# jhhung/kISS

Hardware: AMD Instinct MI355X
Metric: bases/sec suffix_sort (chm13v2.0-size synthetic, k=256) (higher is better)
Workload: dtype u8; 1 GPU; suffix_sort genome-like synthetic n=3117292070 k=256 (stand-in for chm13v2.0.fa, BASELINE.json configs[1]); PARALLEL_SORTING; text resident in HBM, SA left in HBM; n=3117292070, k=256, seed=2, parallelism=single GPU, lms=905939973, lms_rounds=9, tied_after_round0_item_rounds=184319413, big_segment_item_rounds=72866550, workspace_bytes=80357006484, induce_passes=47

## Files before the change

### kiss_amd/csrc/api.hip

```cpp
#include "kiss_internal.hpp"
#include <cstdlib>
#include <chrono>
#include <mutex>
#include <cstring>
#include <new>

KTimer::KTimer(kiss_hip_ctx *c, int cls, uint64_t items) : ctx(c), idx(-1)
{
    if (!((ctx->profile_mask >> cls) & 1ull)) return;
    if (ctx->ev_used == ctx->ev_pool.size()) {
        kiss_hip_ctx::Ev e;
        if (hipEventCreate(&e.a) != hipSuccess || hipEventCreate(&e.b) != hipSuccess) return;
        e.cls = 0;
        ctx->ev_pool.push_back(e);
    }
    idx = (int)ctx->ev_used++;
    ctx->ev_pool[idx].cls = cls;
    ctx->stats.launches_kernel[cls]++;
    ctx->stats.items_kernel[cls] += items;
    (void)hipEventRecord(ctx->ev_pool[idx].a, ctx->stream);
}
KTimer::~KTimer()
{
    if (idx >= 0) (void)hipEventRecord(ctx->ev_pool[idx].b, ctx->stream);
}
void ktimer_collect(kiss_hip_ctx *ctx)
{
    for (size_t i = 0; i < ctx->ev_used; i++) {
        float ms = 0.f;
        if (hipEventElapsedTime(&ms, ctx->ev_pool[i].a, ctx->ev_pool[i].b) == hipSuccess)
            ctx->stats.ms_kernel[ctx->ev_pool[i].cls] += ms;
    }
    ctx->ev_used = 0;
}

static void kiss_opts_supported_from_env(KissOpts &o)
{
    o.debug = getenv("KISS_HIP_DEBUG") != nullptr;
    if (const char *e = getenv("KISS_HIP_XFER_THREADS")) o.xfer_threads = atoi(e);
    if (const char *e = getenv("KISS_HIP_PREFAULT_THREADS")) o.prefault_threads = atoi(e);
}
#ifdef KISS_HIP_HOOKS
static bool env_on(const char *name) { return getenv(name) != nullptr; }
static unsigned long long env_u64(const char *name, unsigned long long dflt)
{
    const char *e = getenv(name);
    return e ? strtoull(e, nullptr, 0) : dflt;
}
void kiss_opts_refresh(kiss_hip_ctx *ctx)
{
    KissOpts o;
    kiss_opts_supported_from_env(o);
    if (const char *e = getenv("KISS_HIP_SYNC_READBACK")) o.sync_readback = atoi(e) != 0;
    o.no_serialize = env_on("KISS_HIP_NO_SERIALIZE");
    o.no_lms_exact = env_on("KISS_HIP_NO_LMS_EXACT");
    o.heads_by_compare = env_on("KISS_HIP_LMS_HEADS_BY_COMPARE");
    o.no_early_out = env_on("KISS_HIP_NO_EARLY_OUT");
    o.no_pivot_rounds = env_on("KISS_HIP_NO_PIVOT_ROUNDS");
    o.pivot_from_round2 = env_on("KISS_HIP_PIVOT_FROM_ROUND2");
    o.pair_keys = env_on("KISS_HIP_PAIR_KEYS");
    o.no_fc0_onepass = env_on("KISS_HIP_NO_FC0_ONEPASS");
    o.no_pair_records = env_on("KISS_HIP_NO_PAIR_RECORDS");
    o.no_small_fused = env_on("KISS_HIP_NO_SMALL_FUSED");
    o.no_class_bytes = env_on("KISS_HIP_NO_CLASS_BYTES");
    o.no_pivot_ctx = env_on("KISS_HIP_NO_PIVOT_CTX");
    o.no_taint = env_on("KISS_HIP_NO_TAINT");
    o.isa_direct = env_on("KISS_HIP_ISA_DIRECT");
    o.no_onesweep = env_on("KISS_HIP_NO_ONESWEEP");
    o.rx_one_tile = env_on("KISS_HIP_RX_ONE_TILE");
    o.merge_lms = env_on("KISS_HIP_MERGE_LMS");
    o.no_small_alphabet = env_on("KISS_HIP_NO_SMALL_ALPHABET");
    o.induce_one_pass = env_on("KISS_HIP_INDUCE_ONE_PASS");
    o.verify = env_on("KISS_HIP_VERIFY");
    o.no_prefault = env_on("KISS_HIP_NO_PREFAULT");
    o.doubling_h0 = (uint32_t)env_u64("KISS_HIP_DOUBLING_H0", 0);
    o.tcap0 = env_u64("KISS_HIP_TCAP0", 0);
    o.pivot_slots = (int)env_u64("KISS_HIP_PIVOT_SLOTS", 3);
    o.small_seg = (uint32_t)env_u64("KISS_HIP_SMALL_SEG", 0);
    o.near_merge_min = (uint32_t)env_u64("KISS_HIP_NEAR_MERGE_MIN", 4096);
    o.induce_small_max = (uint32_t)env_u64("KISS_HIP_INDUCE_SMALL_MAX", 0);
    o.collapse_cap = (uint32_t)env_u64("KISS_HIP_COLLAPSE_CAP", 0);
    o.collapse_n = env_u64("KISS_HIP_COLLAPSE_N", 0);
    o.fm_heavy = (uint32_t)env_u64("KISS_HIP_FM_HEAVY", 0);
    o.fm_light = (uint32_t)env_u64("KISS_HIP_FM_LIGHT", 0);
    o.fm_mm_wave = env_on("KISS_HIP_FM_MM_WAVE");
    o.fm_mm_budget = env_u64("KISS_HIP_FM_MM_BUDGET", 0);
    o.fm8_group = env_on("KISS_HIP_FM8_GROUP");
    o.isa_direct_max = env_u64("KISS_HIP_ISA_DIRECT_MAX", 0);
    o.lx_sync_points = (unsigned)env_u64("KISS_HIP_LX_SYNC_POINTS", 0);
    o.tie_trace = (unsigned)env_u64("KISS_HIP_TIE_TRACE", 0);
    o.poison = (uint32_t)env_u64("KISS_HIP_POISON", 0);
    if (const char *e = getenv("KISS_HIP_DUMP_PIVOT")) snprintf(o.dump_pivot, sizeof o.dump_pivot, "%s", e);
    ctx->opts = o;
}
static std::mutex &kiss_launch_mutex()
// ... 760 lines not shown
        }
    }
    return KISS_HIP_OK;
}

int kiss_hip_debug_radix_sort(kiss_hip_ctx *ctx, uint64_t *keys, uint32_t *pos, uint64_t count, int key_lo_bit)
{
    if (!ctx || !keys || !pos || count > ctx->m_cap) return KISS_HIP_E_INVALID;
    KCHECK(hipSetDevice(ctx->device));
    KCHECK(hipMemcpy(ctx->keyA, keys, count * 8, hipMemcpyHostToDevice));
    KCHECK(hipMemcpy(ctx->posA, pos, count * 4, hipMemcpyHostToDevice));
    RadixBufs rb = kiss_ctx_radix_bufs(ctx);
    int res = 0;
    KTRY(kiss_radix_sort(ctx, rb, count, key_lo_bit, 0, &res));
    KTRY(kiss_radix_check(ctx));
    ktimer_collect(ctx);
    KCHECK(hipMemcpy(keys, rb.key[res], count * 8, hipMemcpyDeviceToHost));
    KCHECK(hipMemcpy(pos, rb.pos[res], count * 4, hipMemcpyDeviceToHost));
    return KISS_HIP_OK;
}

int kiss_hip_debug_fail_alloc_over(kiss_hip_ctx *ctx, uint64_t bytes)
{
    if (!ctx) return KISS_HIP_E_INVALID;
#ifdef KISS_HIP_HOOKS
    ctx->fail_alloc_over = bytes;
    return KISS_HIP_OK;
#else
    (void)bytes;
    return KISS_HIP_E_UNSUPPORTED;
#endif
}

int kiss_hip_has_hooks(void)
{
#ifdef KISS_HIP_HOOKS
    return 1;
#else
    return 0;
#endif
}

int kiss_hip_debug_scan_u32(kiss_hip_ctx *ctx, uint32_t *data, uint64_t count)
{
    if (!ctx || !data || count > ctx->m_cap) return KISS_HIP_E_INVALID;
    KCHECK(hipSetDevice(ctx->device));
    KCHECK(hipMemcpy(ctx->posA, data, count * 4, hipMemcpyHostToDevice));
    KTRY(kiss_scan_u32(ctx, ctx->posA, ctx->posB, count));
    KCHECK(hipStreamSynchronize(ctx->stream));
    KCHECK(hipMemcpy(data, ctx->posB, count * 4, hipMemcpyDeviceToHost));
    return KISS_HIP_OK;
}

int kiss_hip_ctx_get_stage_outputs(kiss_hip_ctx *ctx, uint32_t *lms_ascending, uint32_t *lms_sorted, uint64_t *counts)
{
    if (!ctx) return KISS_HIP_E_INVALID;
    KCHECK(hipSetDevice(ctx->device));
    if (lms_ascending && ctx->m)
        KCHECK(hipMemcpy(lms_ascending, ctx->lms_pos, ctx->m * sizeof(uint32_t), hipMemcpyDeviceToHost));
    if (lms_sorted && ctx->m) {
        KTRY(kiss_merge_lms(ctx));
        KCHECK(hipStreamSynchronize(ctx->stream));
    }
    if (lms_sorted && ctx->m)
        KCHECK(hipMemcpy(lms_sorted, ctx->lmsP, ctx->m * sizeof(uint32_t), hipMemcpyDeviceToHost));
    if (counts)
// ... 22 lines not shown
```

### kiss_amd/csrc/kiss_internal.hpp

```cpp
#pragma once
#include <hip/hip_runtime.h>
#include <stdint.h>
#include <stddef.h>
#include <mutex>
#include <vector>
#include "../../include/kiss_hip.h"

struct KissOpts {
    bool debug = false;
    int xfer_threads = 0;
    int prefault_threads = 0;
    bool sync_readback = false;
    bool no_lms_exact = false;
    bool heads_by_compare = false;
    bool no_early_out = false;
    bool no_pivot_rounds = false;
    bool pivot_from_round2 = false;
    bool pair_keys = false;
    bool no_fc0_onepass = false;
    bool no_pair_records = false;
    bool no_small_fused = false;
    bool no_class_bytes = false;
    bool no_pivot_ctx = false;
    bool no_taint = false;
    bool isa_direct = false;
    bool no_onesweep = false;
    bool rx_one_tile = false;
    bool merge_lms = false;
    bool no_small_alphabet = false;
    bool induce_one_pass = false;
    bool verify = false;
    bool no_prefault = false;
    bool no_serialize = false;
    bool lock_launches = false;
    bool sync_launches = false;
    uint32_t doubling_h0 = 0;
    uint64_t tcap0 = 0;
    int pivot_slots = 3;
    uint32_t small_seg = 0;
    uint32_t near_merge_min = 4096;
    uint32_t induce_small_max = 0;
    uint32_t collapse_cap = 0;
    uint64_t collapse_n = 0;
    uint32_t fm_heavy = 0, fm_light = 0;
    bool fm_mm_wave = false;
    bool fm8_group = false;
    uint64_t fm_mm_budget = 0;
    uint64_t isa_direct_max = 0;
    unsigned lx_sync_points = 0;
    unsigned tie_trace = 0;
    uint32_t poison = 0;
    char dump_pivot[256] = {0};
};
// ... 159 lines not shown
    uint32_t ind_ticket_base = 0;
    uint32_t *d_small = nullptr;
    uint32_t *h_pinned = nullptr;
    uint32_t *h_pub = nullptr;
    uint32_t *d_pub = nullptr;
    uint32_t pub_seq = 0;
    int pub_mode = -1;
    uint64_t *pairs1 = nullptr, *pairs2 = nullptr;
    uint64_t pairs_cap = 0;
    void *fm_pool[FM_SLOT_COUNT] = {};
    uint64_t fm_pool_cap[FM_SLOT_COUNT] = {};
    hipEvent_t fm_ev[6] = {};
    uint32_t *near_idx = nullptr, *near_fin = nullptr, *near_pos = nullptr, *near_tmp = nullptr, *near_tmp2 = nullptr;
    uint64_t near_cap = 0;
    uint8_t *ga_codes = nullptr;
    uint64_t ga_codes_cap = 0;
    uint8_t *refine_heads = nullptr;
    uint8_t *hfar = nullptr, *hmerged = nullptr;
    uint32_t h_depth = 0;
    bool lms_merged = false;
    int near_form = 0;
    const uint32_t *near_sorted = nullptr;
    const uint32_t *rm_fin = nullptr, *rm_pos = nullptr;
    uint32_t rm_E = 0;

    uint8_t *io_S = nullptr;
    uint32_t *io_SA = nullptr;
    uint64_t io_cap = 0;
    uint32_t *early_host_SA = nullptr;
    hipStream_t early_stream = nullptr;
    std::vector<hipEvent_t> early_events;
    size_t early_used = 0;
    uint64_t early_bytes = 0;
    void *xf_pin[16][2] = {};
    hipEvent_t xf_done[16][2] = {};
    hipStream_t xf_stream[16] = {};
    int xf_ready = 0;

    uint64_t n = 0, m = 0, m_far = 0;
    uint64_t counts[12] = {0};
    kiss_hip_stats stats{};
    uint64_t profile_mask = 0;
    struct Ev { hipEvent_t a, b; int cls; };
    std::vector<Ev> ev_pool;
    size_t ev_used = 0;
};

void kiss_drain_deferred(kiss_hip_ctx *ctx);
struct KissOwnStreamAtExit {
    kiss_hip_ctx *ctx;
    explicit KissOwnStreamAtExit(kiss_hip_ctx *c) : ctx(c) {}
    ~KissOwnStreamAtExit()
    {
        if (ctx) ctx->stream = ctx->own_stream;
    }
    KissOwnStreamAtExit(const KissOwnStreamAtExit &) = delete;
    KissOwnStreamAtExit &operator=(const KissOwnStreamAtExit &) = delete;
};
struct KissCallStream : KissOwnStreamAtExit {
    KissCallStream(kiss_hip_ctx *c, void *stream) : KissOwnStreamAtExit(c)
    {
        ctx->stream = stream ? (hipStream_t)stream : ctx->own_stream;
        if (!ctx->deferred_free.empty()) kiss_drain_deferred(ctx);
    }
};

struct KTimer {
    kiss_hip_ctx *ctx;
    int idx;
    KTimer(kiss_hip_ctx *c, int cls, uint64_t items);
    ~KTimer();
};
void ktimer_collect(kiss_hip_ctx *ctx);

static inline uint64_t div_up(uint64_t a, uint64_t b) { return (a + b - 1) / b; }

int kiss_lms_reserve(kiss_hip_ctx *ctx, uint64_t m_cap, uint64_t t_cap_wanted = 0, bool defer_frees = false);
int kiss_lms_reserve_deferred(kiss_hip_ctx *ctx, uint64_t m_cap);
int kiss_tied_reserve(kiss_hip_ctx *ctx, uint64_t t_cap);
int kiss_workspace_ready(kiss_hip_ctx *ctx);
int kiss_need_ctx_words(kiss_hip_ctx *ctx);
int kiss_pack_text(kiss_hip_ctx *ctx, const uint8_t *d_S, uint64_t n);
int kiss_classify(kiss_hip_ctx *ctx, uint64_t n, uint64_t depth , uint64_t win_lo, uint64_t win_hi);
int kiss_readback(kiss_hip_ctx *ctx, const void *d_src, uint32_t nwords);
std::mutex &kiss_device_mutex(int device);
int kiss_scan_u32(kiss_hip_ctx *ctx, const uint32_t *in, uint32_t *out, uint64_t count);
int kiss_scan_u64(kiss_hip_ctx *ctx, const uint64_t *in, uint64_t *out, uint64_t count);
int kiss_zero_u32(kiss_hip_ctx *ctx, void *p, uint64_t count_u32);
int kiss_fill_u32(kiss_hip_ctx *ctx, void *p, uint32_t value, uint64_t count_u32);
struct RadixBufs {
    uint64_t *key[2];
    uint32_t *seg[2];
    uint32_t *pos[2];
    const uint32_t *first_pos = nullptr;
};
static inline RadixBufs kiss_ctx_radix_bufs(kiss_hip_ctx *ctx)
{
    RadixBufs b;
    b.key[0] = ctx->keyA;
    b.key[1] = ctx->keyB;
    b.seg[0] = b.seg[1] = nullptr;
    b.pos[0] = ctx->posA;
    b.pos[1] = ctx->posB;
// ... 11 lines not shown
constexpr uint32_t KISS_EXACT_H0 = 512;
int kiss_exact_refine(kiss_hip_ctx *ctx, uint64_t n, uint32_t h0, uint32_t *d_SA, uint8_t *heads_in = nullptr);
int kiss_isa_build(kiss_hip_ctx *ctx, const uint32_t *SA, uint64_t total, uint32_t *isa);
int kiss_rank_build_lms(kiss_hip_ctx *ctx, const uint32_t *L, const uint32_t *lms_asc, uint64_t m, uint64_t n,
                        uint32_t *rank, uint64_t *pairs1, uint64_t *pairs2, uint32_t *small, uint64_t small_words);
int kiss_lms_exact_refine(kiss_hip_ctx *ctx, uint64_t n, uint32_t h0, uint32_t *scratch, bool *resolved);
int kiss_merge_lms(kiss_hip_ctx *ctx);
#ifdef KISS_HIP_HOOKS
void kiss_tie_trace_report(kiss_hip_ctx *ctx);
#endif
int kiss_place_lms(kiss_hip_ctx *ctx, uint64_t n, uint32_t k, uint64_t depth);
int kiss_xfer_h2d(kiss_hip_ctx *ctx, void *d_dst, const void *h_src, uint64_t bytes);
int kiss_io_reserve(kiss_hip_ctx *ctx, uint64_t n);
int kiss_cached_ctx_run(int device, uint64_t n, int (*fn)(kiss_hip_ctx *, void *), void *arg);
template <class F>
static inline int kiss_one_shot_cached(int device, uint64_t max_n, const F &f)
{
    return kiss_cached_ctx_run(device, max_n, [](kiss_hip_ctx *ctx, void *p) { return (*static_cast<const F *>(p))(ctx); }, (void *)&f);
}
template <class F>
static inline int kiss_one_shot_own(int device, uint64_t max_n, const F &f)
{
    kiss_hip_ctx *ctx = nullptr;
    int rc = kiss_hip_ctx_create(&ctx, device, max_n);
    if (rc) return rc;
    rc = f(ctx);
    kiss_hip_ctx_destroy(ctx);
    return rc;
}
int kiss_xfer_d2h(kiss_hip_ctx *ctx, void *h_dst, const void *d_src, uint64_t bytes);
void kiss_xfer_free(kiss_hip_ctx *ctx);
int kiss_induce(kiss_hip_ctx *ctx, uint64_t n, uint32_t *d_SA);
int kiss_early_out(kiss_hip_ctx *ctx, const uint32_t *d_SA, uint64_t lo, uint64_t hi);

#ifdef __HIPCC__
__device__ __forceinline__ void kiss_words2(const uint64_t *__restrict__ pk, uint64_t w, uint64_t &a, uint64_t &b)
{
    const uint64_t w0 = w & ~1ull;
    const ulonglong2 ab = *reinterpret_cast<const ulonglong2 *>(__builtin_assume_aligned(pk + w0, 16));
    const uint64_t c = pk[w0 + 2];
    const bool odd = (w & 1ull) != 0;
    a = odd ? ab.y : ab.x;
    b = odd ? c : ab.y;
}
__device__ __forceinline__ void kiss_words5(const uint64_t *__restrict__ pk, uint64_t w, uint64_t x[5])
{
    const uint64_t w0 = w & ~1ull;
    const ulonglong2 p0 = *reinterpret_cast<const ulonglong2 *>(__builtin_assume_aligned(pk + w0, 16));
    const ulonglong2 p1 = *reinterpret_cast<const ulonglong2 *>(__builtin_assume_aligned(pk + w0 + 2, 16));
    const ulonglong2 p2 = *reinterpret_cast<const ulonglong2 *>(__builtin_assume_aligned(pk + w0 + 4, 16));
    const bool odd = (w & 1ull) != 0;
    x[0] = odd ? p0.y : p0.x;
    x[1] = odd ? p1.x : p0.y;
    x[2] = odd ? p1.y : p1.x;
    x[3] = odd ? p2.x : p1.y;
    x[4] = odd ? p2.y : p2.x;
}
__device__ __forceinline__ uint64_t kiss_key32(const uint64_t *__restrict__ pk, uint64_t p)
{
    const uint32_t s = (uint32_t)(p & 31u) * 2u;
    uint64_t a, b;
    kiss_words2(pk, p >> 5, a, b);
    return (a << s) | ((b >> 1) >> (63u - s));
}
__device__ __forceinline__ uint32_t kiss_base(const uint64_t *__restrict__ pk, uint64_t p)
{
// ... 39 lines not shown
```

### kiss_amd/csrc/lms_sort.hip

```cpp
#include "flag_compact.hpp"
#include <cstdio>
#include <vector>

using namespace kiss_fc;

namespace {

constexpr uint32_t LMS_SMALL_SEG = 24;
constexpr int ROUND0_BASES = 20;

__global__ __launch_bounds__(LS_THREADS) void k_gather_keys(const uint64_t *__restrict__ pk, uint64_t n,
                                                           const uint32_t *__restrict__ pos, uint64_t count,
                                                           uint64_t depth_off, uint64_t mask,
                                                           uint64_t *__restrict__ key, const uint32_t *__restrict__ seg,
                                                           const uint32_t *__restrict__ segstart, uint32_t min_len,
                                                           uint32_t max_len)
{
    uint64_t i = (uint64_t)blockIdx.x * LS_THREADS + threadIdx.x;
    if (i >= count) return;
    if (seg) {
        const uint32_t sg = seg[i];
        const uint32_t len = segstart[sg + 1] - segstart[sg];
        if (len < min_len || len > max_len) return;
    }
// ... 313 lines not shown
    const int wa = s_a[w], wb = s_b[w];
    uint32_t r;
    bool taint, tied_before;
    if (!s_unsorted[w]) {
        r = (uint32_t)(w - wa);
        tied_before = w > wa && s_inorder[w - 1] == 2;
        taint = tied_before || (w + 1 < wb && s_inorder[w] == 2);
    } else {
        const uint32_t behind = (2u << (wb - 1 - w)) - 2u;
        r = (uint32_t)__popc(~s_before[w] & behind);
        taint = s_tiedm[w] != 0;
        tied_before = false;
        for (int j = wa; j < w; j++) {
            r += (s_before[j] >> (w - j)) & 1u;
            tied_before = tied_before || ((s_tiedm[j] >> (w - j)) & 1u);
        }
        taint = taint || tied_before;
    }
    const uint32_t dst = slot[my_a + r];
    out[dst] = s_pos[w];
    if (hfar && tied_before) hfar[dst] = 0;
    if (tctx) octx[dst] = tctx[i] | (taint ? KISS_CTX_TAINT : 0u);
    else if (taint) octx[dst] = KISS_CTX_TAINT;
    big[i] = 0;
}

__global__ __launch_bounds__(LS_THREADS) void k_pair_finish(const uint64_t *__restrict__ pk, uint64_t n,
                                                           const uint32_t *__restrict__ rpos0,
                                                           const uint32_t *__restrict__ rpos1,
                                                           const uint32_t *__restrict__ rslot, uint64_t npairs,
                                                           uint64_t off, uint64_t depth, uint32_t *__restrict__ out,
                                                           uint32_t *__restrict__ octx, uint8_t *__restrict__ hfar)
{
    const uint64_t i = (uint64_t)blockIdx.x * LS_THREADS + threadIdx.x;
    if (i >= npairs) return;
    const uint32_t p0 = rpos0[i], p1 = rpos1[i], s = rslot[i];
    bool taint = false;
    const bool swap = deep_less(pk, n, p1, p0, off - 32, depth, false, &taint);
    if (!swap && !taint) return;
    const uint32_t c0 = octx[s], c1 = octx[s + 1];
    const uint32_t t = taint ? KISS_CTX_TAINT : 0u;
    if (swap) {
        out[s] = p1;
        out[s + 1] = p0;
    }
    octx[s] = (swap ? c1 : c0) | t;
    octx[s + 1] = (swap ? c0 : c1) | t;
    if (hfar && taint) hfar[s + 1] = 0;
}

__device__ __forceinline__ uint32_t pivot_class(const uint64_t *__restrict__ bkey, uint32_t a, uint32_t b, uint64_t k)
{
    const uint64_t pv = bkey[(a + b) >> 1];
    return k < pv ? 0u : (k == pv ? 1u : 2u);
}

__global__ __launch_bounds__(LS_THREADS) void k_pivot_class(const uint64_t *__restrict__ bkey,
                                                           const uint32_t *__restrict__ bseg,
                                                           const uint32_t *__restrict__ bsegstart, uint64_t nbig,
                                                           uint64_t *__restrict__ cls)
{
    const uint64_t i = (uint64_t)blockIdx.x * LS_THREADS + threadIdx.x;
    if (i >= nbig) return;
    const uint32_t sid = bseg[i];
    const uint32_t c = pivot_class(bkey, bsegstart[sid], bsegstart[sid + 1], bkey[i]);
    cls[i] = c == 0 ? 1ull : (c == 1 ? (1ull << 32) : 0ull);
}

__global__ __launch_bounds__(LS_THREADS) void k_pivot_scatter(const uint64_t *__restrict__ bkey,
                                                             const uint32_t *__restrict__ bpos,
                                                             const uint32_t *__restrict__ bseg,
                                                             const uint32_t *__restrict__ bsegstart, uint64_t nbig,
                                                             const uint64_t *__restrict__ cls,
                                                             const uint64_t *__restrict__ ex,
                                                             const uint64_t *__restrict__ tot,
                                                             uint64_t *__restrict__ okey, uint32_t *__restrict__ opos,
                                                             uint64_t *__restrict__ ne)
{
    const uint64_t i = (uint64_t)blockIdx.x * LS_THREADS + threadIdx.x;
    if (i >= nbig) return;
    const uint32_t sid = bseg[i];
// ... 83 lines not shown
        complete = true;
    }
    key <<= (uint64_t)slotbits * (uint64_t)(slots - used);
    key = (key << 1) | (complete ? 1ull : 0ull);
    keyout[i] = (key << (64 - (slots * slotbits + 1))) | (with_ctx ? (uint64_t)kiss_load_ctx_n(pk, bpos[i], KISS_KEY_CTX_BASES) : 0ull);
}

__global__ __launch_bounds__(LS_THREADS) void k_pivot_heads(const uint64_t *__restrict__ key,
                                                           const uint32_t *__restrict__ seg, uint64_t nbig,
                                                           int complete_bit, uint8_t *__restrict__ heads,
                                                           uint64_t cmp_mask)
{
    const uint64_t i = (uint64_t)blockIdx.x * LS_THREADS + threadIdx.x;
    if (i >= nbig) return;
    const uint64_t k = key[i] & cmp_mask;
    const bool complete = ((k >> complete_bit) & 1ull) != 0;
    const bool same_prev = i > 0 && seg[i] == seg[i - 1] && (key[i - 1] & cmp_mask) == k;
    uint8_t h = 1;
    if (same_prev && !complete) h = 0;
    if (complete && (same_prev || (i + 1 < nbig && seg[i + 1] == seg[i] && (key[i + 1] & cmp_mask) == k))) h |= 2;
    if (complete && same_prev) h |= 4;
    heads[i] = h;
}

__global__ void k_ctx_lengths_anchor(const uint64_t *pk, uint32_t *out)
{
    out[threadIdx.x] = kiss_load_ctx(pk, out[threadIdx.x + 64]);
}


struct LmsViews {
    uint32_t *rpos0, *rpos1, *rslot;
    uint64_t rcol;
    uint64_t *K1;
    uint64_t *key2;
    uint64_t *F1, *F2;
    uint8_t *pivot_heads;
    uint32_t *seg2, *bss;
    uint32_t *sortpos[2];
    uint32_t *tctx, *bslot;
    uint64_t *d_total, *d_ptot;
    uint32_t *d_nbig;
};

LmsViews views_of(kiss_hip_ctx *ctx)
{
    LmsViews v;
    v.rcol = (ctx->m_far / 2 + 4) & ~3ull;
    v.rpos0 = reinterpret_cast<uint32_t *>(ctx->keyA);
    v.rpos1 = v.rpos0 + v.rcol;
    v.rslot = v.rpos1 + v.rcol;
    v.K1 = ctx->keyA;
    v.key2 = ctx->keyB;
    v.F1 = ctx->flags;
    v.F2 = ctx->flags + ctx->t_cap;
    v.pivot_heads = reinterpret_cast<uint8_t *>(ctx->segB);
    v.seg2 = ctx->segB;
    v.bss = ctx->segstartB;
    v.sortpos[0] = ctx->lmsP;
    v.sortpos[1] = ctx->lmsC;
    v.tctx = v.bslot = ctx->bslot;
    v.d_total = reinterpret_cast<uint64_t *>(ctx->d_small + 2);
    v.d_nbig = ctx->d_small + 8;
    v.d_ptot = reinterpret_cast<uint64_t *>(ctx->d_small + 24);
    return v;
}

struct LmsSort {
    kiss_hip_ctx *ctx;
    uint64_t n, depth;
    bool dbg;
    bool pivot_on;
    bool pivot_r1;
    int pivot_slots;
    bool no_pair_keys;
    uint32_t small_seg;
    bool small_fused;
    LmsViews v;
    uint32_t *Pc, *Sc, *Gc, *SSc;
    uint64_t count, nseg;
    uint64_t off = ROUND0_BASES;
    uint64_t npairs = 0;
    bool have_tctx = false;
    bool first_refine = true;
    unsigned pivot_rounds_done = 0;

    FcOut survivors() const { return FcOut{Pc, Sc, Gc, SSc}; }
    void take_tied_arrays()
    {
        Sc = ctx->slotA;
        Gc = ctx->segA;
        SSc = ctx->segstartA;
        v = views_of(ctx);
    }
    void set_survivors(uint64_t tot)
    {
        count = tot >> 32;
        nseg = tot & 0xFFFFFFFFull;
    }
};

struct Round {
// ... 56 lines not shown
            if ((tot >> 32) <= ctx->t_cap) break;
            if (attempt) return KINTERNAL();
            KTRY(regrow_tied(s, tot >> 32));
        }
        s.have_tctx = true;
    } else {
        FcJob job;
        job.key = rb.key[res];
        job.pos = rb.pos[res];
        job.count = count;
        job.cmp_shift = r0_shift;
        job.out = ctx->lms_sorted_far;
        job.octx = ctx->lms_ctx_far;
        KTRY(fc_count(ctx, job, s.v.d_total));
        KTRY(read_u64(ctx, s.v.d_total, &tot));
        if ((tot >> 32) > ctx->t_cap) {
            KTRY(regrow_tied(s, tot >> 32));
            KTRY(fc_count(ctx, job, s.v.d_total));
        }
        job.nctx = s.v.tctx;
        KTRY(fc_compact(ctx, job, s.survivors(), &s.have_tctx));
    }
    s.set_survivors(tot);
    if (s.dbg)
        fprintf(stderr, "[kiss_hip] round 0: items %llu -> survivors %llu in %llu segments\n", (unsigned long long)count,
                (unsigned long long)s.count, (unsigned long long)s.nseg);
    return KISS_HIP_OK;
}

int finish_pair_records(LmsSort &s)
{
    kiss_hip_ctx *ctx = s.ctx;
    if (s.npairs > ctx->m_far / 2) return KINTERNAL();
    {
        KTimer t(ctx, KISS_HIP_K_SEGRANK, 2 * s.npairs);
        hipLaunchKernelGGL(k_pair_finish, dim3((unsigned)div_up(s.npairs, LS_THREADS)), dim3(LS_THREADS), 0, ctx->stream, ctx->pk, s.n,
                           s.v.rpos0, s.v.rpos1, s.v.rslot, s.npairs, (uint64_t)ROUND0_BASES, s.depth, ctx->lms_sorted_far,
                           ctx->lms_ctx_far, ctx->hfar);
        KCHECK(hipGetLastError());
    }
    ctx->stats.pair_records = (uint32_t)s.npairs;
    ctx->stats.sort_item_rounds += 2 * s.npairs;
    if (s.count == 0) ctx->stats.lms_rounds++;
    return KISS_HIP_OK;
}

int gather_keys(LmsSort &s, const Round &r)
{
    kiss_hip_ctx *ctx = s.ctx;
    if (s.small_fused && r.pivot_ahead) return KISS_HIP_OK;
    const uint32_t *seg = s.Gc;
    uint32_t min_len = s.small_seg + 1u, max_len = 0xFFFFFFFFu;
    if (!s.small_fused) {
        seg = s.no_pair_keys ? s.Gc : (const uint32_t *)nullptr;
        min_len = 3u;
        max_len = r.pivot_ahead ? s.small_seg : 0xFFFFFFFFu;
    }
    KTimer t(ctx, KISS_HIP_K_KEYGATHER, s.count);
    set_u32(ctx, s.SSc + s.nseg, (uint32_t)s.count);
    hipLaunchKernelGGL(k_gather_keys, dim3(r.grid), dim3(LS_THREADS), 0, ctx->stream, ctx->pk, s.n, s.Pc, s.count, s.off, r.mask,
                       s.v.K1, seg, s.SSc, min_len, max_len);
    KCHECK(hipGetLastError());
    return KISS_HIP_OK;
}

int finish_small_segments(LmsSort &s, const Round &r)
{
    kiss_hip_ctx *ctx = s.ctx;
    {
        KTimer t(ctx, KISS_HIP_K_SEGRANK, s.count);
        set_u32(ctx, s.SSc + s.nseg, (uint32_t)s.count, s.v.d_nbig);
        const uint32_t *tctx = (s.have_tctx && s.first_refine) ? s.v.tctx : (const uint32_t *)nullptr;
        if (s.small_fused) {
            hipLaunchKernelGGL(k_small_finish, dim3(r.grid), dim3(SF_THREADS), 0, ctx->stream, ctx->pk, s.n, s.Pc, s.Sc, s.Gc, s.SSc,
                               (uint32_t)s.count, s.off, s.depth, r.mask, ctx->lms_sorted_far, r.bigb, tctx, ctx->lms_ctx_far,
                               ctx->hfar);
        } else {
            hipLaunchKernelGGL(k_seg_adjacent, dim3(r.grid), dim3(LS_THREADS), 0, ctx->stream, ctx->pk, s.n, s.v.K1, s.Pc, s.Gc,
                               s.SSc, s.count, s.off, s.depth, s.small_seg, r.inorder);
            hipLaunchKernelGGL(k_seg_finish, dim3(r.grid), dim3(LS_THREADS), 0, ctx->stream, ctx->pk, s.n, s.v.K1, s.Pc, s.Sc, s.Gc,
                               s.SSc, s.count, s.off, s.depth, s.small_seg, r.inorder, ctx->lms_sorted_far, r.bigb, s.v.d_nbig,
                               tctx, ctx->lms_ctx_far, ctx->hfar);
        }
        KCHECK(hipGetLastError());
    }
    ctx->stats.lms_rounds++;
    ctx->stats.sort_item_rounds += s.count;
    return KISS_HIP_OK;
}

int compact_big_segments(LmsSort &s, const Round &r, uint64_t nbig, uint64_t nbigseg)
{
    kiss_hip_ctx *ctx = s.ctx;
    const BigbOut to{ctx->bkeyA, ctx->bposA, ctx->bsegA, s.v.bslot, s.v.bss};
// ... 189 lines not shown
    hipStream_t stream;
    hipEvent_t e0 = nullptr, e1 = nullptr;
    DbgSpan(kiss_hip_ctx *ctx, bool on) : stream(ctx->stream)
    {
        if (!on) return;
        (void)hipEventCreate(&e0);
        (void)hipEventCreate(&e1);
        (void)hipEventRecord(e0, stream);
    }
    float ms()
    {
        float v = 0;
        (void)hipEventRecord(e1, stream);
        (void)hipEventSynchronize(e1);
        (void)hipEventElapsedTime(&v, e0, e1);
        return v;
    }
    ~DbgSpan()
    {
        if (e0) (void)hipEventDestroy(e0);
        if (e1) (void)hipEventDestroy(e1);
    }
};

}

int kiss_lms_sort(kiss_hip_ctx *ctx, uint64_t n, uint32_t k, uint64_t depth)
{
    (void)k;
    const uint64_t m_far = ctx->m_far;
    ctx->stats.lms_rounds = 0;
    ctx->stats.sort_item_rounds = 0;
    ctx->stats.pair_records = 0;
    if (m_far == 0) return KISS_HIP_OK;
    if (m_far == 1) {
        KCHECK(hipMemcpyAsync(ctx->lms_sorted_far, ctx->lms_pos, sizeof(uint32_t), hipMemcpyDeviceToDevice,
                              ctx->stream));
        KTRY(kiss_zero_u32(ctx, ctx->lms_ctx_far, 1));
        return KISS_HIP_OK;
    }
    LmsSort s;
    s.ctx = ctx;
    s.n = n;
    s.depth = depth;
    s.dbg = ctx->opts.debug;
    s.pivot_on = !ctx->opts.no_pivot_rounds;
    s.pivot_r1 = !ctx->opts.pivot_from_round2;
    s.pivot_slots = ctx->opts.pivot_slots >= 1 && ctx->opts.pivot_slots <= 8 ? ctx->opts.pivot_slots : 3;
    s.no_pair_keys = !ctx->opts.pair_keys;
    s.small_seg = ctx->opts.small_seg >= 2 && ctx->opts.small_seg <= 4096 ? ctx->opts.small_seg : LMS_SMALL_SEG;
    s.small_fused = !ctx->opts.no_small_fused && s.small_seg == LMS_SMALL_SEG;
    s.take_tied_arrays();

    KTRY(round0(s));
    if (s.npairs) KTRY(finish_pair_records(s));

    for (;; s.first_refine = false) {
        if (s.count == 0) break;
        if (depth && s.off >= depth) return KINTERNAL();
        const Round r = round_of(s);
        KTRY(gather_keys(s, r));
        uint64_t bt;
        {
            DbgSpan span(ctx, s.dbg);
            KTRY(finish_small_segments(s, r));
            KTRY(bigb_count(ctx, r.bigb, s.count, s.v.d_total, &bt));
            if (s.dbg) fprintf(stderr, "[kiss_hip]   seg_finish + flag scan %.3f ms\n", span.ms());
        }
        const uint64_t nbig = bt >> 32, nbigseg = bt & 0xFFFFFFFFull;
        if (s.dbg)
            fprintf(stderr, "[kiss_hip] round off=%llu: items %llu in %llu segments, big-segment items %llu\n",
                    (unsigned long long)s.off, (unsigned long long)s.count, (unsigned long long)s.nseg, (unsigned long long)nbig);
        if (nbig == 0) break;
        KTRY(compact_big_segments(s, r, nbig, nbigseg));
        if (r.pivot_ahead) {
            KTRY(pivot_round(s, nbig, nbigseg));
            continue;
        }
        SortedBig sorted;
        if (uint64_t *NE = class_split_flags(s, nbig)) KTRY(class_split_round(s, r, NE, nbig, nbigseg, &sorted));
        else KTRY(radix_round(s, r, nbig, nbigseg, &sorted));
        KTRY(closing_compaction(s, r, sorted, nbig));
        s.off += 32;
        if (!depth && s.off > n + 64 && s.count > 0) return KINTERNAL();
        if (!depth && s.off >= KISS_EXACT_MSD_MAX_DEPTH && s.count > 0) return KISS_INTERNAL_TOO_DEEP;
    }
    return KISS_HIP_OK;
}
```

### kiss_amd/csrc/xfer.hip

```cpp
#include "kiss_internal.hpp"
#include <atomic>
#include <cstdlib>
#include <cstring>
#include <new>
#include <thread>
#include <vector>

namespace {

constexpr int XF_MAX_THREADS = 16;
static int xf_threads(const kiss_hip_ctx *ctx)
{
    const int v = ctx->opts.xfer_threads ? ctx->opts.xfer_threads : 8;
    return v < 1 ? 1 : (v > XF_MAX_THREADS ? XF_MAX_THREADS : v);
}
#define XF_THREADS xf_threads(ctx)
constexpr size_t XF_CHUNK = 16ull << 20;

bool host_is_pinned(const void *p)
{
    hipPointerAttribute_t a;
    std::memset(&a, 0, sizeof a);
    if (hipPointerGetAttributes(&a, p) != hipSuccess) {
        (void)hipGetLastError();
// ... 86 lines not shown
            th.emplace_back(work, t);
        } catch (...) {
            orphan.push_back(t);
        }
    }
    if (threads > 0) work(0);
    for (int t : orphan) work(t);
    for (auto &x : th) x.join();
    return status;
}

}

int kiss_early_out(kiss_hip_ctx *ctx, const uint32_t *d_SA, uint64_t lo, uint64_t hi)
{
    if (!ctx->early_host_SA || hi <= lo) return KISS_HIP_OK;
    if (!ctx->early_stream) KCHECK(hipStreamCreateWithFlags(&ctx->early_stream, hipStreamNonBlocking));
    if (ctx->early_used == ctx->early_events.size()) {
        hipEvent_t e;
        KCHECK(hipEventCreateWithFlags(&e, hipEventDisableTiming));
        ctx->early_events.push_back(e);
    }
    hipEvent_t ev = ctx->early_events[ctx->early_used++];
    KCHECK(hipEventRecord(ev, ctx->stream));
    KCHECK(hipStreamWaitEvent(ctx->early_stream, ev, 0));
    KCHECK(hipMemcpyAsync(ctx->early_host_SA + lo, d_SA + lo, (hi - lo) * sizeof(uint32_t), hipMemcpyDeviceToHost,
                          ctx->early_stream));
    ctx->early_bytes += (hi - lo) * sizeof(uint32_t);
    return KISS_HIP_OK;
}

bool kiss_host_is_pinned(const void *p) { return host_is_pinned(p); }

#include <sys/mman.h>
#include <unistd.h>
#ifndef MADV_POPULATE_WRITE
#define MADV_POPULATE_WRITE 23
#endif
struct kiss_prefault {
    std::vector<std::thread> th;
    std::atomic<bool> stop{false};
};

static bool looks_untouched(uint64_t lo, uint64_t hi, uint64_t page)
{
    const uint64_t pages = (hi - lo) / page;
    unsigned missing = 0, asked = 0;
    for (uint64_t i = 0; i < 64; i++) {
        const uint64_t q = lo + (pages * i / 64) * page;
        unsigned char vec = 0;
        if (mincore((void *)(uintptr_t)q, (size_t)page, &vec) != 0) return false;
        asked++;
        missing += (vec & 1u) ? 0u : 1u;
    }
    return asked && missing * 2 > asked;
}

void *kiss_prefault_start(kiss_hip_ctx *ctx, void *p, uint64_t bytes)
{
    if (ctx->opts.no_prefault || bytes < (64ull << 20)) return nullptr;
    const uint64_t page = (uint64_t)sysconf(_SC_PAGESIZE);
    const uint64_t lo = ((uint64_t)(uintptr_t)p + page - 1) / page * page, hi = ((uint64_t)(uintptr_t)p + bytes) / page * page;
    if (hi <= lo || !looks_untouched(lo, hi, page)) return nullptr;
    kiss_prefault *h = new (std::nothrow) kiss_prefault;
    if (!h) return nullptr;
    int T = 4;
    if (ctx->opts.prefault_threads >= 1 && ctx->opts.prefault_threads <= 64) T = ctx->opts.prefault_threads;
    const uint64_t pages = (hi - lo) / page, per = (pages + (uint64_t)T - 1) / (uint64_t)T;
    for (int t = 0; t < T; t++) {
        const uint64_t a = lo + (uint64_t)t * per * page, b = a + per * page < hi ? a + per * page : hi;
        if (a >= b) break;
        try {
            h->th.emplace_back([a, b, h] {
                const uint64_t step = 64ull << 20;
                for (uint64_t q = a; q < b && !h->stop.load(std::memory_order_relaxed); q += step)
                    if (madvise((void *)(uintptr_t)q, (size_t)((b - q) < step ? (b - q) : step), MADV_POPULATE_WRITE) != 0) return;
            });
        } catch (...) {
            break;
        }
    }
    return h;
}

void kiss_prefault_join(void *handle)
{
    kiss_prefault *h = static_cast<kiss_prefault *>(handle);
    if (!h) return;
    h->stop.store(true, std::memory_order_relaxed);
    for (auto &t : h->th) t.join();
    delete h;
}

void kiss_xfer_free(kiss_hip_ctx *ctx)
{
    for (hipEvent_t e : ctx->early_events) (void)hipEventDestroy(e);
    ctx->early_events.clear();
    if (ctx->early_stream) (void)hipStreamDestroy(ctx->early_stream);
    ctx->early_stream = nullptr;
    for (int t = 0; t < XF_MAX_THREADS; t++) {
        for (int b = 0; b < 2; b++) {
            if (ctx->xf_pin[t][b]) (void)hipHostFree(ctx->xf_pin[t][b]);
            if (ctx->xf_done[t][b]) (void)hipEventDestroy(ctx->xf_done[t][b]);
            ctx->xf_pin[t][b] = nullptr;
            ctx->xf_done[t][b] = nullptr;
        }
        if (ctx->xf_stream[t]) (void)hipStreamDestroy(ctx->xf_stream[t]);
        ctx->xf_stream[t] = nullptr;
    }
    ctx->xf_ready = false;
}

int kiss_xfer_h2d(kiss_hip_ctx *ctx, void *d_dst, const void *h_src, uint64_t bytes)
{
    if (!bytes) return KISS_HIP_OK;
    if (host_is_pinned(h_src) || bytes < (1u << 20)) {
        KCHECK(hipMemcpyAsync(d_dst, h_src, bytes, hipMemcpyHostToDevice, ctx->stream));
        KCHECK(hipStreamSynchronize(ctx->stream));
        return KISS_HIP_OK;
    }
    return xfer_staged(ctx, d_dst, const_cast<void *>(h_src), bytes, true);
}

int kiss_xfer_d2h(kiss_hip_ctx *ctx, void *h_dst, const void *d_src, uint64_t bytes)
{
    if (!bytes) return KISS_HIP_OK;
    if (host_is_pinned(h_dst) || bytes < (1u << 20)) {
        KCHECK(hipMemcpyAsync(h_dst, d_src, bytes, hipMemcpyDeviceToHost, ctx->stream));
        KCHECK(hipStreamSynchronize(ctx->stream));
        return KISS_HIP_OK;
    }
    return xfer_staged(ctx, const_cast<void *>(d_src), h_dst, bytes, false);
// ... 2 lines not shown
```

Measured before the change: 46.91 billion bases/s.

## Run pair-finish kernel on a low-priority side stream overlapping later rounds

Moves the k_pair_finish kernel (deep comparison of tied pairs after round 0) onto a separate low-priority stream, forked via an event and joined only when the key buffer is next written or at the end of the LMS sort. The kernel becomes grid-stride with the grid capped at one workgroup per CU, so it occupies a small slice of the GPU while the main-stream rounds proceed. The intent is to hide the latency of the deep pair comparisons behind subsequent sort rounds. It adds cross-stream synchronization and a risk of contention, and the early join before key gathering may limit how much overlap is possible.

```diff
diff --git a/kiss_amd/csrc/api.hip b/kiss_amd/csrc/api.hip
--- a/kiss_amd/csrc/api.hip
+++ b/kiss_amd/csrc/api.hip
@@ -5,7 +5,7 @@
 #include <cstring>
 #include <new>
 
-KTimer::KTimer(kiss_hip_ctx *c, int cls, uint64_t items) : ctx(c), idx(-1)
+KTimer::KTimer(kiss_hip_ctx *c, int cls, uint64_t items, hipStream_t on) : ctx(c), idx(-1), stream(on ? on : c->stream)
 {
     if (!((ctx->profile_mask >> cls) & 1ull)) return;
     if (ctx->ev_used == ctx->ev_pool.size()) {
@@ -18,11 +18,11 @@
     ctx->ev_pool[idx].cls = cls;
     ctx->stats.launches_kernel[cls]++;
     ctx->stats.items_kernel[cls] += items;
-    (void)hipEventRecord(ctx->ev_pool[idx].a, ctx->stream);
+    (void)hipEventRecord(ctx->ev_pool[idx].a, stream);
 }
 KTimer::~KTimer()
 {
-    if (idx >= 0) (void)hipEventRecord(ctx->ev_pool[idx].b, ctx->stream);
+    if (idx >= 0) (void)hipEventRecord(ctx->ev_pool[idx].b, stream);
 }
 void ktimer_collect(kiss_hip_ctx *ctx)
 {
@@ -61,6 +61,9 @@
     o.pair_keys = env_on("KISS_HIP_PAIR_KEYS");
     o.no_fc0_onepass = env_on("KISS_HIP_NO_FC0_ONEPASS");
     o.no_pair_records = env_on("KISS_HIP_NO_PAIR_RECORDS");
+    o.pair_serial = env_on("KISS_HIP_PAIR_SERIAL");
+    o.pair_low_priority = env_u64("KISS_HIP_PAIR_PRIORITY", KISS_PAIR_LOW_PRIORITY) != 0;
+    o.pair_wgs_per_cu = (uint32_t)env_u64("KISS_HIP_PAIR_WGS_PER_CU", KISS_PAIR_WGS_PER_CU);
     o.no_small_fused = env_on("KISS_HIP_NO_SMALL_FUSED");
     o.no_class_bytes = env_on("KISS_HIP_NO_CLASS_BYTES");
     o.no_pivot_ctx = env_on("KISS_HIP_NO_PIVOT_CTX");
@@ -887,6 +890,10 @@
 #endif
 }
 
+#ifdef KISS_HIP_HOOKS
+int kiss_hip_debug_pair_join_point(kiss_hip_ctx *ctx) { return ctx ? ctx->pair_join_point : KISS_HIP_E_INVALID; }
+#endif
+
 int kiss_hip_has_hooks(void)
 {
 #ifdef KISS_HIP_HOOKS
diff --git a/kiss_amd/csrc/kiss_internal.hpp b/kiss_amd/csrc/kiss_internal.hpp
--- a/kiss_amd/csrc/kiss_internal.hpp
+++ b/kiss_amd/csrc/kiss_internal.hpp
@@ -6,6 +6,8 @@
 #include <vector>
 #include "../../include/kiss_hip.h"
 
+#define KISS_PAIR_LOW_PRIORITY 1
+#define KISS_PAIR_WGS_PER_CU 1
 struct KissOpts {
     bool debug = false;
     int xfer_threads = 0;
@@ -19,6 +21,9 @@
     bool pair_keys = false;
     bool no_fc0_onepass = false;
     bool no_pair_records = false;
+    bool pair_serial = false;
+    bool pair_low_priority = KISS_PAIR_LOW_PRIORITY != 0;
+    uint32_t pair_wgs_per_cu = KISS_PAIR_WGS_PER_CU;
     bool no_small_fused = false;
     bool no_class_bytes = false;
     bool no_pivot_ctx = false;
@@ -244,6 +249,12 @@
     std::vector<hipEvent_t> early_events;
     size_t early_used = 0;
     uint64_t early_bytes = 0;
+    hipStream_t pair_stream = nullptr;
+    hipEvent_t pair_fork_ev = nullptr, pair_join_ev = nullptr;
+    bool pair_stream_low = false;
+    bool pair_stream_refused = false;
+    int pair_cus = 0;
+    int pair_join_point = 0;
     void *xf_pin[16][2] = {};
     hipEvent_t xf_done[16][2] = {};
     hipStream_t xf_stream[16] = {};
@@ -280,7 +291,8 @@
 struct KTimer {
     kiss_hip_ctx *ctx;
     int idx;
-    KTimer(kiss_hip_ctx *c, int cls, uint64_t items);
+    hipStream_t stream;
+    KTimer(kiss_hip_ctx *c, int cls, uint64_t items, hipStream_t on = nullptr);
     ~KTimer();
 };
 void ktimer_collect(kiss_hip_ctx *ctx);
@@ -358,6 +370,7 @@
 void kiss_xfer_free(kiss_hip_ctx *ctx);
 int kiss_induce(kiss_hip_ctx *ctx, uint64_t n, uint32_t *d_SA);
 int kiss_early_out(kiss_hip_ctx *ctx, const uint32_t *d_SA, uint64_t lo, uint64_t hi);
+bool kiss_pair_stream(kiss_hip_ctx *ctx, bool low);
 
 #ifdef __HIPCC__
 __device__ __forceinline__ void kiss_words2(const uint64_t *__restrict__ pk, uint64_t w, uint64_t &a, uint64_t &b)
diff --git a/kiss_amd/csrc/lms_sort.hip b/kiss_amd/csrc/lms_sort.hip
--- a/kiss_amd/csrc/lms_sort.hip
+++ b/kiss_amd/csrc/lms_sort.hip
@@ -369,21 +369,21 @@
                                                            uint64_t off, uint64_t depth, uint32_t *__restrict__ out,
                                                            uint32_t *__restrict__ octx, uint8_t *__restrict__ hfar)
 {
-    const uint64_t i = (uint64_t)blockIdx.x * LS_THREADS + threadIdx.x;
-    if (i >= npairs) return;
-    const uint32_t p0 = rpos0[i], p1 = rpos1[i], s = rslot[i];
-    bool taint = false;
-    const bool swap = deep_less(pk, n, p1, p0, off - 32, depth, false, &taint);
-    if (!swap && !taint) return;
-    const uint32_t c0 = octx[s], c1 = octx[s + 1];
-    const uint32_t t = taint ? KISS_CTX_TAINT : 0u;
-    if (swap) {
-        out[s] = p1;
-        out[s + 1] = p0;
-    }
-    octx[s] = (swap ? c1 : c0) | t;
-    octx[s + 1] = (swap ? c0 : c1) | t;
-    if (hfar && taint) hfar[s + 1] = 0;
+    for (uint64_t i = (uint64_t)blockIdx.x * LS_THREADS + threadIdx.x; i < npairs; i += (uint64_t)gridDim.x * LS_THREADS) {
+        const uint32_t p0 = rpos0[i], p1 = rpos1[i], s = rslot[i];
+        bool taint = false;
+        const bool swap = deep_less(pk, n, p1, p0, off - 32, depth, false, &taint);
+        if (!swap && !taint) continue;
+        const uint32_t c0 = octx[s], c1 = octx[s + 1];
+        const uint32_t t = taint ? KISS_CTX_TAINT : 0u;
+        if (swap) {
+            out[s] = p1;
+            out[s + 1] = p0;
+        }
+        octx[s] = (swap ? c1 : c0) | t;
+        octx[s + 1] = (swap ? c0 : c1) | t;
+        if (hfar && taint) hfar[s + 1] = 0;
+    }
 }
 
 __device__ __forceinline__ uint32_t pivot_class(const uint64_t *__restrict__ bkey, uint32_t a, uint32_t b, uint64_t k)
@@ -533,7 +533,7 @@
 struct LmsViews {
     uint32_t *rpos0, *rpos1, *rslot;
     uint64_t rcol;
-    uint64_t *K1;
+    const uint64_t *K1;
     uint64_t *key2;
     uint64_t *F1, *F2;
     uint8_t *pivot_heads;
@@ -567,8 +567,33 @@
     return v;
 }
 
+struct PairFork {
+    kiss_hip_ctx *ctx;
+    bool pending = false;
+    explicit PairFork(kiss_hip_ctx *c) : ctx(c) { ctx->pair_join_point = 0; }
+    int join(int where)
+    {
+        if (!pending) return KISS_HIP_OK;
+        pending = false;
+        ctx->pair_join_point = where;
+        const hipError_t e = hipStreamWaitEvent(ctx->stream, ctx->pair_join_ev, 0);
+        if (e != hipSuccess) (void)hipStreamSynchronize(ctx->pair_stream);
+        KCHECK(e);
+        return KISS_HIP_OK;
+    }
+    ~PairFork()
+    {
+        if (!pending) return;
+        (void)join(0);
+        (void)hipStreamSynchronize(ctx->pair_stream);
+    }
+    PairFork(const PairFork &) = delete;
+    PairFork &operator=(const PairFork &) = delete;
+};
+
 struct LmsSort {
     kiss_hip_ctx *ctx;
+    PairFork *fork = nullptr;
     uint64_t n, depth;
     bool dbg;
     bool pivot_on;
@@ -691,16 +716,39 @@
 {
     kiss_hip_ctx *ctx = s.ctx;
     if (s.npairs > ctx->m_far / 2) return KINTERNAL();
-    {
-        KTimer t(ctx, KISS_HIP_K_SEGRANK, 2 * s.npairs);
-        hipLaunchKernelGGL(k_pair_finish, dim3((unsigned)div_up(s.npairs, LS_THREADS)), dim3(LS_THREADS), 0, ctx->stream, ctx->pk, s.n,
+    const bool beside = !ctx->opts.pair_serial && kiss_pair_stream(ctx, ctx->opts.pair_low_priority) &&
+                        hipEventRecord(ctx->pair_fork_ev, ctx->stream) == hipSuccess &&
+                        hipStreamWaitEvent(ctx->pair_stream, ctx->pair_fork_ev, 0) == hipSuccess;
+    const hipStream_t on = beside ? ctx->pair_stream : ctx->stream;
+    uint64_t grid = div_up(s.npairs, LS_THREADS);
+    const uint64_t cap = (uint64_t)ctx->opts.pair_wgs_per_cu * (uint64_t)ctx->pair_cus;
+    if (beside && cap && grid > cap) grid = cap;
+    hipError_t launched;
+    {
+        KTimer t(ctx, KISS_HIP_K_SEGRANK, 2 * s.npairs, on);
+        hipLaunchKernelGGL(k_pair_finish, dim3((unsigned)grid), dim3(LS_THREADS), 0, on, ctx->pk, s.n,
                            s.v.rpos0, s.v.rpos1, s.v.rslot, s.npairs, (uint64_t)ROUND0_BASES, s.depth, ctx->lms_sorted_far,
                            ctx->lms_ctx_far, ctx->hfar);
-        KCHECK(hipGetLastError());
-    }
+        launched = hipGetLastError();
+    }
+    if (beside) {
+        s.fork->pending = true;
+        if (hipEventRecord(ctx->pair_join_ev, ctx->pair_stream) != hipSuccess) {
+            (void)hipStreamSynchronize(ctx->pair_stream);
+            s.fork->pending = false;
+        }
+    }
+    KCHECK(launched);
     ctx->stats.pair_records = (uint32_t)s.npairs;
     ctx->stats.sort_item_rounds += 2 * s.npairs;
     if (s.count == 0) ctx->stats.lms_rounds++;
+    return KISS_HIP_OK;
+}
+
+int keys_for_writing(LmsSort &s, uint64_t **K1)
+{
+    KTRY(s.fork->join(1));
+    *K1 = s.ctx->keyA;
     return KISS_HIP_OK;
 }
 
@@ -715,10 +763,12 @@
         min_len = 3u;
         max_len = r.pivot_ahead ? s.small_seg : 0xFFFFFFFFu;
     }
+    uint64_t *K1;
+    KTRY(keys_for_writing(s, &K1));
     KTimer t(ctx, KISS_HIP_K_KEYGATHER, s.count);
     set_u32(ctx, s.SSc + s.nseg, (uint32_t)s.count);
     hipLaunchKernelGGL(k_gather_keys, dim3(r.grid), dim3(LS_THREADS), 0, ctx->stream, ctx->pk, s.n, s.Pc, s.count, s.off, r.mask,
-                       s.v.K1, seg, s.SSc, min_len, max_len);
+                       K1, seg, s.SSc, min_len, max_len);
     KCHECK(hipGetLastError());
     return KISS_HIP_OK;
 }
@@ -974,6 +1024,7 @@
     ctx->stats.lms_rounds = 0;
     ctx->stats.sort_item_rounds = 0;
     ctx->stats.pair_records = 0;
+    PairFork fork(ctx);
     if (m_far == 0) return KISS_HIP_OK;
     if (m_far == 1) {
         KCHECK(hipMemcpyAsync(ctx->lms_sorted_far, ctx->lms_pos, sizeof(uint32_t), hipMemcpyDeviceToDevice,
@@ -993,6 +1044,7 @@
     s.small_seg = ctx->opts.small_seg >= 2 && ctx->opts.small_seg <= 4096 ? ctx->opts.small_seg : LMS_SMALL_SEG;
     s.small_fused = !ctx->opts.no_small_fused && s.small_seg == LMS_SMALL_SEG;
     s.take_tied_arrays();
+    s.fork = &fork;
 
     KTRY(round0(s));
     if (s.npairs) KTRY(finish_pair_records(s));
@@ -1027,5 +1079,5 @@
         if (!depth && s.off > n + 64 && s.count > 0) return KINTERNAL();
         if (!depth && s.off >= KISS_EXACT_MSD_MAX_DEPTH && s.count > 0) return KISS_INTERNAL_TOO_DEEP;
     }
-    return KISS_HIP_OK;
-}
+    return fork.join(2);
+}
diff --git a/kiss_amd/csrc/xfer.hip b/kiss_amd/csrc/xfer.hip
--- a/kiss_amd/csrc/xfer.hip
+++ b/kiss_amd/csrc/xfer.hip
@@ -142,6 +142,37 @@
 
 bool kiss_host_is_pinned(const void *p) { return host_is_pinned(p); }
 
+static void pair_stream_free(kiss_hip_ctx *ctx)
+{
+    if (ctx->pair_stream) (void)hipStreamDestroy(ctx->pair_stream);
+    if (ctx->pair_fork_ev) (void)hipEventDestroy(ctx->pair_fork_ev);
+    if (ctx->pair_join_ev) (void)hipEventDestroy(ctx->pair_join_ev);
+    ctx->pair_stream = nullptr;
+    ctx->pair_fork_ev = ctx->pair_join_ev = nullptr;
+}
+
+bool kiss_pair_stream(kiss_hip_ctx *ctx, bool low)
+{
+    if (ctx->pair_stream_refused) return false;
+    if (ctx->pair_stream && ctx->pair_stream_low == low) return true;
+    pair_stream_free(ctx);
+    int least = 0, greatest = 0, cus = 0;
+    bool ok = hipDeviceGetStreamPriorityRange(&least, &greatest) == hipSuccess &&
+              hipDeviceGetAttribute(&cus, hipDeviceAttributeMultiprocessorCount, ctx->device) == hipSuccess && cus > 0;
+    ok = ok && hipStreamCreateWithPriority(&ctx->pair_stream, hipStreamNonBlocking, low ? least : 0) == hipSuccess;
+    ok = ok && hipEventCreateWithFlags(&ctx->pair_fork_ev, hipEventDisableTiming) == hipSuccess;
+    ok = ok && hipEventCreateWithFlags(&ctx->pair_join_ev, hipEventDisableTiming) == hipSuccess;
+    if (!ok) {
+        (void)hipGetLastError();
+        pair_stream_free(ctx);
+        ctx->pair_stream_refused = true;
+        return false;
+    }
+    ctx->pair_stream_low = low;
+    ctx->pair_cus = cus;
+    return true;
+}
+
 #include <sys/mman.h>
 #include <unistd.h>
 #ifndef MADV_POPULATE_WRITE
@@ -208,6 +239,7 @@
     ctx->early_events.clear();
     if (ctx->early_stream) (void)hipStreamDestroy(ctx->early_stream);
     ctx->early_stream = nullptr;
+    pair_stream_free(ctx);
     for (int t = 0; t < XF_MAX_THREADS; t++) {
         for (int b = 0; b < 2; b++) {
             if (ctx->xf_pin[t][b]) (void)hipHostFree(ctx->xf_pin[t][b]);
```

Result: no change. 47.57 billion bases/s, median of 6 (+1.4%).
